# joesharratt1229/DT4Image_Restoration

Hardware: AMD Instinct MI355X
Metric: pnp_admm_iterations_per_sec (higher is better)
Workload: dtype f32

## Files before the change

### dt4image_restoration_amd/csrc/conv_kernels.hip

```cpp
#include "pnp_internal.h"
#include "conv_staging.h"
#include <cstring>
#include <cstdlib>

namespace pnp {



const LayerSpec kLayers[N_LAYERS] = {
    {2, 32, 3, 0, SRC_SIGMA, 0},    {32, 32, 3, 0, SRC_PLAIN, 0},   {32, 32, 3, 0, SRC_PLAIN, 0},
    {32, 64, 3, 1, SRC_POOL, 0},    {64, 64, 3, 1, SRC_PLAIN, 0},   {64, 64, 3, 1, SRC_PLAIN, 0},
    {64, 128, 3, 2, SRC_POOL, 0},   {128, 128, 3, 2, SRC_PLAIN, 0}, {128, 128, 3, 2, SRC_PLAIN, 0},
    {128, 256, 3, 3, SRC_POOL, 0},  {256, 256, 3, 3, SRC_PLAIN, 0}, {256, 256, 3, 3, SRC_PLAIN, 0},
    {256, 512, 3, 4, SRC_POOL, 0},  {512, 512, 3, 4, SRC_PLAIN, 0}, {512, 512, 3, 4, SRC_PLAIN, 0},
    {768, 256, 3, 3, SRC_UPCAT, 256}, {256, 256, 3, 3, SRC_PLAIN, 0}, {256, 256, 3, 3, SRC_PLAIN, 0},
    {384, 128, 3, 2, SRC_UPCAT, 128}, {128, 128, 3, 2, SRC_PLAIN, 0}, {128, 128, 3, 2, SRC_PLAIN, 0},
    {192, 64, 3, 1, SRC_UPCAT, 64},  {64, 64, 3, 1, SRC_PLAIN, 0},   {64, 64, 3, 1, SRC_PLAIN, 0},
    {96, 32, 3, 0, SRC_UPCAT, 32},   {32, 32, 3, 0, SRC_PLAIN, 0},   {32, 32, 3, 0, SRC_PLAIN, 0},
    {32, 1, 1, 0, SRC_PLAIN, 0},
};

ConvPlan conv3x3_plan(int N, int H, int W, int Cin, int Cout, bool bf16, int src_mode, bool allow_ws) {
    ConvPlan p{};
    p.tw = W >= 32 ? 32 : (W >= 16 ? 16 : 8);
// ... 613 lines not shown
    if (blocks > 2048u) blocks = 2048u;
    hipLaunchKernelGGL(splitk_reduce_kernel, dim3(blocks), dim3(256), 0, s, a.partial, a.bias, a.dst, a.tact, plane4,
                       p.splitk, a.Cout / 4, (size_t)a.H * a.W * a.Cout / 4);
    return hipGetLastError();
}

bool conv3x3_tensor_fits(int N, int H, int W, int Cin, int Cout) {
    (void)Cin;
    return (size_t)N * H * W * (size_t)Cout * 4 < ((size_t)1 << 31);
}

bool conv3x3_pooled_output_ok(const ConvPlan& p) {
    return p.splitk == 1 && p.mt <= 2 && p.nt == 1 && p.wm == 4;
}

size_t conv3x3_partial_floats(const ConvPlan& p, int N, int H, int W, int Cout) {
    return (p.mt <= 2 && p.wn >= 2) ? (size_t)p.splitk * N * H * W * Cout : 0;
}

Tuning tuning_from_env() {
    Tuning t;
    if (const char* v = getenv("PNP_WINO_MIN_CIN")) t.wino_min_cin = atoi(v);
    if (const char* v = getenv("PNP_WINO_MIN_BLOCKS")) t.wino_min_blocks = atol(v);
    t.wino_big = getenv("PNP_WINO_BIG_GROUPS") != nullptr;
    t.wino_small = getenv("PNP_WINO_SMALL_GROUPS") != nullptr;
    t.no_wino = getenv("PNP_NO_WINOGRAD") != nullptr;
    if (const char* v = getenv("PNP_WINO_F4_MIN_CIN")) t.f4_min_cin = atoi(v);
    t.no_f4 = getenv("PNP_NO_WINO_F4") != nullptr;
    t.no_f4_phased = getenv("PNP_NO_WINO_F4_PHASED") != nullptr;
    t.no_f4_fused_last = getenv("PNP_NO_F4_FUSED_LAST") != nullptr;
    t.no_f4_fused_first = getenv("PNP_NO_F4_FUSED_FIRST") != nullptr;
    if (const char* v = getenv("PNP_WINO_F4_MT16")) t.f4_mt16 = atoi(v);
    if (const char* v = getenv("PNP_WINO_F4_CS")) t.f4_cs = atoi(v);
    if (const char* v = getenv("PNP_WINO_F4_ORDER")) t.f4_order = atoi(v) != 0;
    t.bf16_f32_acts = getenv("PNP_BF16_F32_ACTS") != nullptr;
    t.bf16_no_ws = getenv("PNP_BF16_NO_WS") != nullptr;
    t.bf16_w1 = getenv("PNP_BF16_W1") != nullptr;
    t.bf16_no_holdhi = getenv("PNP_BF16_NO_HOLDHI") != nullptr;
    if (const char* v = getenv("PNP_SLICE128_MIN_N")) t.slice128_min_n = atoi(v);
    if (const char* v = getenv("PNP_TV_NAIVE")) t.tv_naive = atoi(v) != 0;
    if (const char* v = getenv("PNP_HAAR_NAIVE")) t.haar_naive = atoi(v) != 0;
    if (const char* v = getenv("PNP_NCSENSE_COIL_BLOCK")) t.ncsense_block = atoi(v);
    if (const char* v = getenv("PNP_NCSENSE_NAIVE")) t.ncsense_naive = atoi(v) != 0 ? 1 : 0;
    if (const char* v = getenv("PNP_TOEPLITZ_NAIVE")) t.toeplitz_naive = atoi(v) != 0;
    if (const char* v = getenv("PNP_OFFRES_SEG_BLOCK")) t.offres_block = atoi(v);
    if (const char* v = getenv("PNP_OFFRES_GRID_FILTER")) t.offres_grid_filter = atoi(v) != 0;
    if (const char* v = getenv("PNP_FIELDMAP_NAIVE")) t.fieldmap_naive = atoi(v) != 0;
    if (const char* v = getenv("PNP_OFFRES_NAIVE")) t.offres_naive = atoi(v) != 0 ? 1 : 0;
    return t;
}

hipError_t raise_lds_cap(const void* fn, int bytes, DeviceOnce& once) {
    int dev = 0;
    hipError_t e = hipGetDevice(&dev);
    if (e != hipSuccess) return e;
    const uint64_t bit = 1ull << (dev & 63);
    if (once.mask.load(std::memory_order_relaxed) & bit) return hipSuccess;
    e = hipFuncSetAttribute(fn, hipFuncAttributeMaxDynamicSharedMemorySize, bytes);
    if (e != hipSuccess) return e;
    once.mask.fetch_or(bit, std::memory_order_relaxed);
    return hipSuccess;
}

__global__ __launch_bounds__(256) void conv_first_kernel(const float* __restrict__ ximg, const float2* __restrict__ z,
                                                         const float2* __restrict__ u, const float* __restrict__ sigma,
                                                         const float* __restrict__ tact, const float* __restrict__ w,
// ... 172 lines not shown
```

### dt4image_restoration_amd/csrc/pnp_internal.h

```cpp
#pragma once
#include <hip/hip_runtime.h>
#include <stdint.h>
#include <stddef.h>
#include <atomic>
#include <vector>

namespace pnp {

struct Tuning {
    int wino_min_cin = 32;
    long wino_min_blocks = 192;
    bool wino_big = false;
    bool wino_small = false;
    bool no_wino = false;
    int f4_min_cin = 32;
    bool no_f4 = false;
    bool no_f4_fused_first = false;
    bool no_f4_fused_last = false;
    bool no_f4_phased = false;
    int f4_mt16 = 0;
    bool bf16_no_ws = false;
    bool bf16_f32_acts = false;
    bool bf16_no_holdhi = false;
    bool bf16_w1 = false;
    int f4_cs = 1;
    int f4_order = 1;
    int slice128_min_n = 192;
    bool tv_naive = false;
    bool haar_naive = false;
    int ncsense_block = 0;
    int ncsense_naive = -1;
    bool toeplitz_naive = false;
    int offres_block = 0;
    bool offres_grid_filter = false;
    bool fieldmap_naive = false;
    int offres_naive = -1;
};
Tuning tuning_from_env();

struct DeviceOnce { std::atomic<uint64_t> mask{0}; };
hipError_t raise_lds_cap(const void* fn, int bytes, DeviceOnce& once);

enum SrcMode : int { SRC_PLAIN = 0, SRC_SIGMA = 1, SRC_POOL = 2, SRC_UPCAT = 3, SRC_FIRST = 4 };

struct LayerSpec {
    int cin, cout, ksize, level, src, cskip;
};
static constexpr int N_LAYERS = 28;
extern const LayerSpec kLayers[N_LAYERS];

struct ConvArgs {
    const float* src0;
    const float* src1;
    const float* wpack;
    const float* bias;
    float* dst;
    float* pooled;
    const float* last_w; const float* last_b; const float* last_ximg; const float2* last_z; const float2* last_u; float* last_out;
// ... 14 lines not shown
    int diag;
#endif
};

struct ConvPlan {
    int tw, th;
    int bm, bn;
    int mt, nt, wm, wn;
    int ck;
    int splitk;
    int ws;
    int holdhi = 1;
    int tiles_x, tiles_y;
};
ConvPlan conv3x3_plan(int N, int H, int W, int Cin, int Cout, bool bf16 = false, int src_mode = SRC_PLAIN, bool allow_ws = true);
hipError_t launch_conv3x3_bf16ws(const ConvArgs& a, const ConvPlan& p, int src_mode, hipStream_t s);
size_t conv3x3_partial_floats(const ConvPlan& p, int N, int H, int W, int Cout);
bool conv3x3_pooled_output_ok(const ConvPlan& p);
bool conv3x3_tensor_fits(int N, int H, int W, int Cin, int Cout);
hipError_t launch_conv3x3(const ConvArgs& a, const ConvPlan& p, int src_mode, hipStream_t s);

size_t conv3x3_pack_floats(int cin, int cout);
void pack_conv3x3_weights(const float* oihw, int cin, int cout, int ck, float* dst);
size_t conv3x3_pack_floats_bf16(int cin, int cout, int terms);
void pack_conv3x3_weights_bf16(const float* oihw, int cin, int cout, int ck, int terms, float* dst);

struct WinoPlan {
    bool use;
    int algo;
    int tw, th, bn, wm, wn, ck, tiles_x, tiles_y;
    int stack;
    int mt;
    int phased;
    int cs;
    int order;
};
WinoPlan winograd_plan(int N, int H, int W, int Cin, int Cout, int src_mode, const Tuning& t, int Cskip = 0);
bool upsample_lines_regular(int H);
size_t winograd4_pack_floats(int cin, int cout);
void pack_winograd4_weights(const float* oihw, int cin, int cout, int ck, float* dst);
hipError_t launch_conv3x3_winograd4(const ConvArgs& a, const WinoPlan& p, int src_mode, hipStream_t s);
size_t winograd_pack_floats(int cin, int cout);
void pack_winograd_weights(const float* oihw, int cin, int cout, int ck, float* dst);
hipError_t launch_conv3x3_winograd(const ConvArgs& a, const WinoPlan& p, int src_mode, hipStream_t s);

hipError_t launch_conv_first(const float* ximg, const float2* z, const float2* u, const float* sigma,
                             const float* tact, const float* w, const float* bias, float* dst,
                             int N, int H, int W, hipStream_t s, bool dst_bf16 = false);
hipError_t launch_conv_last(const float* act, const float* ximg, const float2* z, const float2* u,
                            const float* tact, const float* w, const float* bias, float* out,
                            int N, int H, int W, hipStream_t s);
hipError_t launch_nhwc_to_nchw(const float* src, float* dst, int N, int C, int H, int W, hipStream_t s);

struct FftPlan {
    int h, w;
    float2* tw_h;
    float2* tw_w;
};

bool kspace_len_ok(int L);
hipError_t launch_fft_rows(const float2* in, float2* out, const float2* tw, int batch, int H, int W, int inverse, int shift, hipStream_t s);
hipError_t launch_fft_cols(float2* data, const float2* tw, int batch, int H, int W, int inverse, int shift, hipStream_t s);
hipError_t launch_fft_rows_real(const float* x, float2* work, const float2* tw, int N, int H, int W, hipStream_t s);
hipError_t launch_fft_rows_fwd_admm(const float* x, const float2* u, float2* work, const float2* tw, const float* tact, int N, int H, int W,
                                    hipStream_t s);
hipError_t launch_fft_cols_prox(float2* work, const float2* tw, const float2* y0s, const uint8_t* masks, int mask_n, const float* mu,
// ... 254 lines not shown
```

### dt4image_restoration_amd/csrc/winograd4_kernels.hip

```cpp
#include "pnp_internal.h"
#include "conv_staging.h"
#include <type_traits>

namespace pnp {

#ifdef PNP_STAMPS
#define W4_SLOTS 32
#define W4_WGS 1024
#define W4_N 16
__device__ unsigned long long g_w4_stamps[W4_SLOTS * W4_WGS * W4_N];
static int g_w4_slot = 0;
#define W4T() __builtin_amdgcn_s_memtime()
#endif

namespace {
constexpr double kA = 0.75, kB = 1.5;
constexpr float fA = 0.75f, fB = 1.5f, fA2 = 0.5625f, fB2 = 2.25f, fA3 = 0.421875f, fB3 = 3.375f;
constexpr float fK0 = 1.265625f;
constexpr float fK1 = 2.8125f;

__device__ __forceinline__ float4 f4add(float4 a, float4 b) { return make_float4(a.x + b.x, a.y + b.y, a.z + b.z, a.w + b.w); }
typedef float v2f __attribute__((ext_vector_type(2)));
typedef float f32x4 __attribute__((ext_vector_type(4)));

// ... 160 lines not shown
    const int g = (isrow ? ty0 : tx0) + pq - 1;
    float4 e = make_float4(0.f, 0.f, 0.f, 0.f);
    if (g >= 0 && g < (isrow ? a.H : a.W)) {
        const float sc = (isrow ? a.rh : a.rw) * (float)g;
        const int i0 = (int)sc;
        const int i1 = i0 + (i0 < (isrow ? Hs : Ws) - 1 ? 1 : 0);
        const float l = fminf(fmaxf(sc - (float)i0, 0.f), 1.f);
        if (isrow) {
            const int s0 = ylo + (pq >> 1);
            const float w0 = 1.f - l, w1 = l;
            e.x = (i0 == s0 ? w0 : 0.f) + (i1 == s0 ? w1 : 0.f);
            e.y = (i0 == s0 + 1 ? w0 : 0.f) + (i1 == s0 + 1 ? w1 : 0.f);
        } else {
            e = make_float4(__int_as_float((i0 - xlo) * LP), __int_as_float((i1 - xlo) * LP), 1.f - l, l);
        }
    }
    *reinterpret_cast<float4*>(&(isrow ? rowT : colT)[4 * pq]) = e;
}

template <int CTRL>
__device__ __forceinline__ float dpp_xchg(float v) {
    return __builtin_bit_cast(float, __builtin_amdgcn_update_dpp(0, __builtin_bit_cast(int, v), CTRL, 0xF, 0xF, false));
}
template <int H, int CTRL>
__device__ __forceinline__ void row_reduce_scatter_step(v2f* P, bool bit) {
#pragma unroll
    for (int i = 0; i < H; ++i) {
        const v2f lo = P[i], hi = P[i + H];
        const v2f keep = bit ? hi : lo, send = bit ? lo : hi;
        P[i] = v2f{keep.x + dpp_xchg<CTRL>(send.x), keep.y + dpp_xchg<CTRL>(send.y)};
    }
}

template <int TW, bool STK, int MT = 32, bool FUSE = false>
__device__ __forceinline__ void wino4_epilogue(const ConvArgs& a, const f32x4 (&acc)[36], int n, int th, int tg, int cl, int cb,
                                               int tx0, int ty0, bool live, float* xch = nullptr) {
    constexpr int TC = TW / 4, TR = MT / TC;
    constexpr unsigned OOB = 0x80000000u;
    const int cout0 = cb * 16 + cl;
    const float bias = a.bias[cout0];
    const int Hp = a.H >> 1, Wp = a.W >> 1;
    auto at6 = [&](v2f m0, v2f m1, v2f m2, v2f m3, v2f m4, v2f m5, v2f* t) {
        const v2f s1 = m1 + m2, d1 = m1 - m2, s2 = m3 + m4, d2 = m3 - m4;
        t[0] = m0 + s1 + s2;
        t[1] = fA * d1 + fB * d2;
        t[2] = fA2 * s1 + fB2 * s2;
        t[3] = fA3 * d1 + fB3 * d2 + m5;
    };
    if (!live) return;
    const bool fused = FUSE && a.last_w != nullptr;
#ifdef PNP_DIAG
    const bool nostore = (a.diag & 1) != 0;
#else
    constexpr bool nostore = false;
#endif
    v2f part[2];
    const __amdgpu_buffer_rsrc_t rdst = __builtin_amdgcn_make_buffer_rsrc(
        (void*)(a.dst + (size_t)(n + (STK ? th : 0)) * a.H * a.W * a.Cout), 0, nostore ? 0 : a.H * a.W * a.Cout * 4, 0x00020000);
    const __amdgpu_buffer_rsrc_t rpool = __builtin_amdgcn_make_buffer_rsrc(
        (void*)(a.pooled != nullptr ? a.pooled + (size_t)(n + (STK ? th : 0)) * Hp * Wp * a.Cout : a.dst), 0,
        (a.pooled != nullptr && !nostore) ? Hp * Wp * a.Cout * 4 : 0, 0x00020000);
#pragma unroll
    for (int rp = 0; rp < 2; ++rp) {
        v2f T[4][6];
#pragma unroll
        for (int j = 0; j < 6; ++j) {
            v2f m[6];
#pragma unroll
            for (int i = 0; i < 6; ++i) m[i] = v2f{acc[6 * i + j][2 * rp], acc[6 * i + j][2 * rp + 1]};
            v2f t[4];
            at6(m[0], m[1], m[2], m[3], m[4], m[5], t);
#pragma unroll
            for (int ay = 0; ay < 4; ++ay) T[ay][j] = t[ay];
        }
        v2f Y[4][4];
#pragma unroll
        for (int ay = 0; ay < 4; ++ay) {
            at6(T[ay][0], T[ay][1], T[ay][2], T[ay][3], T[ay][4], T[ay][5], Y[ay]);
#pragma unroll
            for (int ax = 0; ax < 4; ++ax) {
                const v2f sv = Y[ay][ax] + bias;
                Y[ay][ax] = v2f{fmaxf(sv.x, kLeaky * sv.x), fmaxf(sv.y, kLeaky * sv.y)};
            }
        }
        if constexpr (FUSE) {
            if (fused) {
                const float wl = a.last_w[cout0];
                v2f P[16];
#pragma unroll
                for (int i = 0; i < 16; ++i) P[i] = Y[i >> 2][i & 3] * wl;
                row_reduce_scatter_step<8, 0x140>(P, (cl & 8) != 0);
                row_reduce_scatter_step<4, 0x141>(P, (cl & 4) != 0);
                row_reduce_scatter_step<2, 0x1B>(P, (cl & 2) != 0);
                row_reduce_scatter_step<1, 0xB1>(P, (cl & 1) != 0);
                part[rp] = P[0];
                continue;
            }
        }
#pragma unroll
        for (int e = 0; e < 2; ++e) {
            const int t = 16 * th + 4 * tg + 2 * rp + e;
            const int tr = t / TC;
            const int py = STK ? 4 * (tr % (TR / 2)) : 4 * tr, px = 4 * (t % TC);
            const int gy = ty0 + py, gx = tx0 + px;
            const unsigned base = (gx < a.W) ? (unsigned)(((gy * a.W + gx) * a.Cout + cout0) * 4) : OOB;
            const unsigned rowb = (unsigned)(a.W * a.Cout * 4);
#pragma unroll
// ... 12 lines not shown
#pragma unroll
                    for (int wx = 0; wx < 2; ++wx) {
                        const v2f mx = __builtin_elementwise_max(__builtin_elementwise_max(Y[2 * wy][2 * wx], Y[2 * wy][2 * wx + 1]),
                                                                 __builtin_elementwise_max(Y[2 * wy + 1][2 * wx], Y[2 * wy + 1][2 * wx + 1]));
                        const float val = e == 0 ? mx.x : mx.y;
                        __builtin_amdgcn_raw_buffer_store_b32(__builtin_bit_cast(unsigned, val), rpool, pbase + wy * prowb, wx * a.Cout * 4, 0);
                    }
            }
        }
    }
    if constexpr (FUSE) {
        if (fused) {
            const int cq = cb & 1, lane = 16 * tg + cl;
            float4* const x4 = reinterpret_cast<float4*>(xch) + th * 64 + lane;
            if (cq == 1) *x4 = make_float4(part[0].x, part[0].y, part[1].x, part[1].y);
            __syncthreads();
            if (cq == 0) {
                const float4 o = *x4;
                const float sum[4] = {part[0].x + o.x, part[0].y + o.y, part[1].x + o.z, part[1].y + o.w};
                const float lb = a.last_b[0];
#pragma unroll
                for (int r = 0; r < 4; ++r) {
                    const int t = 16 * th + 4 * tg + r;
                    const int gy = ty0 + 4 * (t / TC) + (cl >> 2), gx = tx0 + 4 * (t % TC) + (cl & 3);
                    if (gy < a.H && gx < a.W && !nostore) {
                        const size_t qx = ((size_t)n * a.H + gy) * a.W + gx;
                        const float img = a.last_ximg != nullptr ? a.last_ximg[qx] : (a.last_z[qx].x - a.last_u[qx].x);
                        a.last_out[qx] = fminf(fmaxf(img + sum[r] + lb, 0.f), 1.f);
                    }
                }
            }
        }
    }
}

template <int TW, int SRC, bool STK = false, int WN = 2, int MT = 32>
__global__ __launch_bounds__(8 * MT * WN, 2) void conv3x3_wino4_kernel(const ConvArgs a) {
    constexpr int CK = 8 * WN, CKP = CK, LP = CK, PPP = CK / 4, NT_ = 8 * MT * WN;
    constexpr int CKQ = WN == 2 ? CK + 4 : CK + 2;
    constexpr int HCN = CK / 2;
    constexpr int TC = TW / 4, TR = MT / TC;
    constexpr int TH = 4 * TR;
    constexpr int SUBH = STK ? TH / 2 + 2 : 0;
    constexpr int PH = STK ? 2 * SUBH : TH + 2, PW = TW + 2;
    constexpr int ITEMS = PH * PW * PPP;
    static_assert(!STK || (TW == 16 && SRC == SRC_PLAIN && WN == 2 && MT == 32), "stacked slices: 16-wide tiles, plain source");
    static_assert(MT == 32 || (MT == 16 && WN == 2), "16-tile M-blocks: 64-channel workgroups only");
    constexpr int NIT = (ITEMS + NT_ - 1) / NT_;
    constexpr bool UP2 = SRC == SRC_UPCAT;
    constexpr bool FIRST = SRC == SRC_FIRST;
    constexpr int LH = TH / 2 + 3, LW = TW / 2 + 3;
    constexpr int LITEMS = LH * LW * PPP;
    constexpr int NITL = (LITEMS + NT_ - 1) / NT_;
    constexpr bool SPLIT = UP2 && WN == 2;
    constexpr int NH0 = SPLIT ? (NIT + 1) / 2 : NIT;
    constexpr int NRAW = SPLIT ? (NH0 > NITL ? NH0 : NITL) : ((UP2 && NITL > NIT) ? NITL : NIT);
    constexpr int S = CK / 4;
    constexpr int PF = WN == 2 ? 9 : 12;
    constexpr int KEEP = WN == 1 ? 6 : 3;
    constexpr int PLANE = MT * CKP;
    static_assert(SRC == SRC_PLAIN || SRC == SRC_UPCAT || SRC == SRC_FIRST, "pooled sources go through the pooled copy");
    static_assert(!FIRST || (WN == 1 && MT == 32), "fused first layer: the 32-channel variant");
    static_assert(36 % PF == 0 && MT * HCN * 2 == NT_, "one (tile, 2-channel, column group) transform item per thread");

    extern __shared__ __attribute__((aligned(16))) float smem[];
    float* const patch = smem;
// ... 291 lines not shown
            }
#ifdef PNP_DIAG
            if ((a.diag & 4) && (xi & 1)) continue;
#endif
            if (xi + PF < 36 + KEEP) bq[xi % PF] = bfrag(bp, bf0, xi + PF);
        }
#ifdef PNP_STAMPS
        { const unsigned long long t = W4T(); st_mfma += t - st_tmp; }
#endif
        if (c + 1 < nchunks) {
            if constexpr (FIRST) first_patch(c + 1);
            else park(c + 1, SPLIT ? 1 : 0);
        }
    }
#ifdef PNP_STAMPS
    st_loop1 = W4T();
    st_tmp = st_loop1;
#endif

    wino4_epilogue<TW, STK, MT, WN == 1 && MT == 32 && SRC == SRC_PLAIN>(a, acc, n, th, tg, cl, cb, tx0, ty0, STK ? (th == 0 ? live0 : live1) : true, smem);
#ifdef PNP_STAMPS
    {
        const int w = (int)blockIdx.x - (int)(gridDim.x / 2);
        if (tid == 0 && w >= 0 && w < W4_WGS && a.stamp_slot < W4_SLOTS) {
            unsigned long long* o = g_w4_stamps + ((size_t)a.stamp_slot * W4_WGS + w) * W4_N;
            const unsigned long long te = W4T();
            o[0] = 1; o[1] = st_setup - st_t0; o[2] = st_commit; o[3] = st_trans; o[4] = st_mfma; o[5] = st_loop1 - st_loop0;
            o[6] = te - st_tmp; o[7] = 0; o[8] = te - st_loop1; o[9] = te - st_t0; o[10] = (unsigned long long)nchunks;
        }
    }
#endif
}

template <int TW, bool STK>
__global__ __launch_bounds__(512, 2) void conv3x3_wino4p_kernel(const ConvArgs a) {
    constexpr int CK = 16, CKP = 16, PPP = 4, NT_ = 512, S = 4;
    constexpr int TC = TW / 4, TR = 32 / TC;
    constexpr int TH = 4 * TR;
    constexpr int SUBH = STK ? TH / 2 + 2 : 0;
    constexpr int PH = STK ? 2 * SUBH : TH + 2, PW = TW + 2;
    constexpr int NPIX = PH * PW, ITEMS = NPIX * PPP;
    constexpr int NIT = (ITEMS + NT_ - 1) / NT_;
    constexpr int PLSZ = ((NPIX * 4 + 15) / 16) * 16 + 4;
    constexpr int PATCH = 4 * PLSZ;
    constexpr int PF = 12, KEEP = 3;
    constexpr int PLANE = 32 * CKP;
    constexpr unsigned OOB = 0x80000000u;
    static_assert(!STK || TW == 16, "stacked slices: 16-wide tiles");
    static_assert((2 * PATCH + 36 * PLANE) * 4 <= 160 * 1024, "two patch copies + V in one CU's LDS");

    extern __shared__ __attribute__((aligned(16))) float smem[];
    float* const patch = smem;
    float* const V = smem + 2 * PATCH;
#ifdef PNP_STAMPS
    unsigned long long st_t0 = W4T(), st_setup = 0, st_loop0 = 0, st_commit = 0, st_trans = 0, st_mfma = 0, st_loop1 = 0, st_tmp = 0;
#endif
    const int tid = threadIdx.x, lane = tid & 63;
    const int wid = __builtin_amdgcn_readfirstlane(tid >> 6);
    const int grp = wid >> 2, cq = wid & 3;
    const int th = grp;
    const int tg = lane >> 4, cl = lane & 15;

    const int ny = a.Cout / 64;
    const int bid = blockIdx.x;
    const int ntl = a.tilesX * a.tilesY * (STK ? (a.N + 1) / 2 : a.N);
    int cby, bt;
    wino4_decode(bid, ny, ntl, a.order, cby, bt);
    if (bt >= ntl) return;
    const int tx0 = (bt % a.tilesX) * TW;
    bt /= a.tilesX;
    const int ty0 = (bt % a.tilesY) * TH;
    const int n = STK ? 2 * (bt / a.tilesY) : bt / a.tilesY;
    const int nsl = STK ? (n + 1 < a.N ? 2 : 1) : 1;
    const bool live0 = !(a.tact != nullptr && a.tact[n] > 0.5f);
    const bool live1 = STK && nsl == 2 && !(a.tact != nullptr && a.tact[n + 1] > 0.5f);
    if (!live0 && !live1) return;
    const int cb = cby * 4 + cq;
    const int nchunks = a.Cin / CK;

    const __amdgpu_buffer_rsrc_t rsrc0 = __builtin_amdgcn_make_buffer_rsrc(
        (void*)(a.src0 + (size_t)n * a.H * a.W * a.Cin), 0, nsl * a.H * a.W * a.Cin * 4, 0x00020000);
    unsigned voff[NIT];
#pragma unroll
    for (int k = 0; k < NIT; ++k) {
        const int idx = tid + k * NT_;
        const int part = idx % PPP, pp = idx / PPP;
        const int py = pp / PW, px = pp % PW;
        const int sub = STK ? py / SUBH : 0;
        const int gy = STK ? py % SUBH - 1 : ty0 + py - 1, gx = tx0 + px - 1;
        voff[k] = (idx < ITEMS && sub < nsl && gy >= 0 && gy < a.H && gx >= 0 && gx < a.W)
                      ? (unsigned)((((sub * a.H + gy) * a.W + gx) * a.Cin + part * 4) * 4) : OOB;
    }
    const int ldst = (tid & 3) * PLSZ + (tid >> 2) * 4;
    float4 raw[NIT];
    auto issue = [&](int c) {
        const int soff = c * CK * 4;
#pragma unroll
        for (int k = 0; k < NIT; ++k)
            raw[k] = __builtin_bit_cast(float4, __builtin_amdgcn_raw_buffer_load_b128(rsrc0, voff[k], soff, 0));
    };
    auto park = [&](int c) {
        float* const dst = patch + (c & 1) * PATCH + ldst;
#pragma unroll
        for (int k = 0; k < NIT; ++k)
            if (tid + k * NT_ < ITEMS) *reinterpret_cast<float4*>(&dst[k * (NT_ / PPP) * 4]) = raw[k];
    };

    auto swz = [](int t16, int g) { return g ^ ((4 - (t16 >> 2)) & 3); };
    const int tgi = tid & 255;
    const int hc = tgi & 7, t16 = (tgi >> 3) & 15;
    const int tj = (wid >> 1) & 1;
    const int tq = 16 * grp + t16;
    const int trow = tq / TC;
    const int wrow = STK ? (trow / (TR / 2)) * SUBH + 4 * (trow % (TR / 2)) : 4 * trow;
    const int win = (hc >> 1) * PLSZ + (wrow * PW + 4 * (tq % TC)) * 4 + 2 * (hc & 1);
    const int vout = tq * CKP + 4 * swz(t16, hc >> 1) + 2 * (hc & 1);

    f32x4 acc[36];
#pragma unroll
    for (int k = 0; k < 36; ++k) acc[k] = f32x4{0.f, 0.f, 0.f, 0.f};

    const size_t stream = (size_t)nchunks * 36 * 64 + kW4Tail / S;
    const float4* const bptr = reinterpret_cast<const float4*>(a.wpack) + (size_t)cb * stream + lane;
    float4 bq[PF];
#pragma unroll
    for (int p = 0; p < KEEP; ++p) bq[p] = bptr[p * 64];
    const int aoff = (16 * th + cl) * CKP + 4 * swz(cl, tg);

    constexpr bool PARK_T = !STK;
    issue(0);
    park(0);
    if constexpr (!PARK_T) { if (grp == 1 && nchunks > 1) { issue(1); park(1); } }
#ifdef PNP_STAMPS
    st_setup = W4T();
    st_loop0 = st_setup;
#endif
    if (grp == 1) __syncthreads();
    for (int c = 0; c < nchunks; ++c) {
#ifdef PNP_STAMPS
        st_tmp = W4T();
#endif
        __syncthreads();
#ifdef PNP_STAMPS
        { const unsigned long long t = W4T(); st_commit += t - st_tmp; st_tmp = t; }
#endif
        if constexpr (PARK_T) { if (c + 1 < nchunks) issue(c + 1); }
        __builtin_amdgcn_s_setprio(3);
        {
            const float* const w = patch + (c & 1) * PATCH + win;
            if (tj == 0) wino4_input_transform<0, PW, 4, PLANE>(w, V + vout);
            else wino4_input_transform<1, PW, 4, PLANE>(w, V + vout);
        }
        __builtin_amdgcn_s_setprio(0);
        __builtin_amdgcn_sched_barrier(0);
        const float4* bp = bptr + (size_t)c * 36 * 64;
#pragma unroll
        for (int p = KEEP; p < PF; ++p) bq[p] = bp[p * 64];
        const int nx = c + 1 + grp;
        if constexpr (PARK_T) { if (c + 1 < nchunks) park(c + 1); }
        else { if (nx < nchunks) issue(nx); }
        __syncthreads();
#ifdef PNP_STAMPS
        { const unsigned long long t = W4T(); st_trans += t - st_tmp; st_tmp = t; }
#endif

        float4 ar[3];
        ar[0] = *reinterpret_cast<const float4*>(&V[aoff]);
        ar[1] = *reinterpret_cast<const float4*>(&V[PLANE + aoff]);
#pragma unroll
        for (int xi = 0; xi < 36; ++xi) {
            if (xi + 2 < 36) ar[(xi + 2) % 3] = *reinterpret_cast<const float4*>(&V[(xi + 2) * PLANE + aoff]);
            __builtin_amdgcn_sched_barrier(0);
            const float4 a0 = ar[xi % 3], b0 = bq[xi % PF];
            acc[xi] = __builtin_amdgcn_mfma_f32_16x16x4f32(a0.x, b0.x, acc[xi], 0, 0, 0);
            acc[xi] = __builtin_amdgcn_mfma_f32_16x16x4f32(a0.y, b0.y, acc[xi], 0, 0, 0);
            acc[xi] = __builtin_amdgcn_mfma_f32_16x16x4f32(a0.z, b0.z, acc[xi], 0, 0, 0);
            acc[xi] = __builtin_amdgcn_mfma_f32_16x16x4f32(a0.w, b0.w, acc[xi], 0, 0, 0);
            __builtin_amdgcn_sched_barrier(0);
#ifdef PNP_DIAG
            if ((a.diag & 4) && (xi & 1)) continue;
#endif
            if (xi + PF < 36 + KEEP) bq[xi % PF] = bp[(xi + PF) * 64];
        }
#ifdef PNP_STAMPS
        { const unsigned long long t = W4T(); st_mfma += t - st_tmp; }
#endif
        if constexpr (!PARK_T) { if (nx < nchunks) park(nx); }
    }
    if (grp == 0) __syncthreads();
#ifdef PNP_STAMPS
    st_loop1 = W4T();
    st_tmp = st_loop1;
#endif

    wino4_epilogue<TW, STK>(a, acc, n, th, tg, cl, cb, tx0, ty0, STK ? (th == 0 ? live0 : live1) : true);
#ifdef PNP_STAMPS
    {
        const int w = (int)blockIdx.x - (int)(gridDim.x / 2);
        if (tid == 0 && w >= 0 && w < W4_WGS && a.stamp_slot < W4_SLOTS) {
            unsigned long long* o = g_w4_stamps + ((size_t)a.stamp_slot * W4_WGS + w) * W4_N;
            const unsigned long long te = W4T();
            o[0] = 1; o[1] = st_setup - st_t0; o[2] = st_commit; o[3] = st_trans; o[4] = st_mfma; o[5] = st_loop1 - st_loop0;
            o[6] = te - st_tmp; o[7] = 0; o[8] = te - st_loop1; o[9] = te - st_t0; o[10] = (unsigned long long)nchunks;
        }
    }
#endif
}

template <int TW, int SRC>
__global__ __launch_bounds__(512, 2) void conv3x3_wino4c_kernel(const ConvArgs a) {
    constexpr int CK = 16, CKP = 16, PPP = 4, NT_ = 512, S = 4, MT = 16;
    constexpr bool UP2 = SRC == SRC_UPCAT;
    static_assert(SRC == SRC_PLAIN || SRC == SRC_UPCAT, "plain or upsample + concat source");
    constexpr int TC = TW / 4, TR = MT / TC;
    constexpr int TH = 4 * TR;
    constexpr int PH = TH + 2, PW = TW + 2;
    constexpr int NPIX = PH * PW, ITEMS = NPIX * PPP;
    constexpr int NIT = (ITEMS + NT_ - 1) / NT_;
    constexpr int PLSZ = ((NPIX * 4 + 15) / 16) * 16 + 4;
    constexpr int PATCH = 4 * PLSZ;
    constexpr int PF = 12, KEEP = 3;
    constexpr int PLANE = MT * CKP;
    constexpr int VSZ = 36 * PLANE;
    constexpr unsigned OOB = 0x80000000u;
    static_assert(NIT == 3 && ITEMS <= NIT * NT_, "three staging items per thread");
    constexpr int LP = CK;
    constexpr int LH = TH / 2 + 3, LW = TW / 2 + 3;
    constexpr int LITEMS = LH * LW * PPP, NITL = (LITEMS + NT_ - 1) / NT_;
// ... 200 lines not shown

    wino4_epilogue<TW, false, 16>(a, acc, n, 0, tg, cl, cb, tx0, ty0, true);
#ifdef PNP_STAMPS
    {
        const int w = (int)blockIdx.x - (int)(gridDim.x / 2);
        if (tid == 0 && w >= 0 && w < W4_WGS && a.stamp_slot < W4_SLOTS) {
            unsigned long long* o = g_w4_stamps + ((size_t)a.stamp_slot * W4_WGS + w) * W4_N;
            const unsigned long long te = W4T();
            o[0] = 1; o[1] = st_setup - st_t0; o[2] = st_commit; o[3] = st_trans; o[4] = st_mfma; o[5] = st_loop1 - st_loop0;
            o[6] = te - st_tmp; o[7] = 0; o[8] = te - st_loop1; o[9] = te - st_t0; o[10] = (unsigned long long)nchunks;
        }
    }
#endif
}

template <int TW, int SRC>
static hipError_t launch_wino4c_inst(const ConvArgs& a, const WinoPlan& p, hipStream_t s) {
    constexpr int TC = TW / 4, TR = 16 / TC, TH = 4 * TR;
    constexpr int NPIX = (TH + 2) * (TW + 2);
    constexpr int PLSZ = ((NPIX * 4 + 15) / 16) * 16 + 4;
    constexpr size_t lowres_f = SRC == SRC_UPCAT ? (size_t)2 * (TH / 2 + 3) * (TW / 2 + 3) * 16 + 4 * (TH + 2 + TW + 2) : 0;
    constexpr size_t lds = ((size_t)2 * 4 * PLSZ + (size_t)2 * 36 * 16 * 16 + lowres_f) * sizeof(float);
    if (p.th != TH || p.tw != TW) return hipErrorInvalidValue;
    if (SRC == SRC_UPCAT && a.Cskip < 3 * 16) return hipErrorInvalidValue;
    auto kern = conv3x3_wino4c_kernel<TW, SRC>;
    static DeviceOnce cap;
    if (hipError_t e = raise_lds_cap((const void*)kern, (int)lds, cap); e != hipSuccess) return e;
    const int ntiles = p.tiles_x * p.tiles_y * a.N, ny = a.Cout / 128;
    dim3 grid((unsigned)(((ntiles + 7) / 8) * 8 * ny));
    hipLaunchKernelGGL(kern, grid, dim3(512), lds, s, a);
    return hipGetLastError();
}

template <int TW, bool STK>
static hipError_t launch_wino4p_inst(const ConvArgs& a, const WinoPlan& p, hipStream_t s) {
    constexpr int TC = TW / 4, TR = 32 / TC, TH = 4 * TR;
    constexpr int NPIX = (STK ? TH + 4 : TH + 2) * (TW + 2);
    constexpr int PLSZ = ((NPIX * 4 + 15) / 16) * 16 + 4;
    constexpr size_t lds = ((size_t)2 * 4 * PLSZ + (size_t)36 * 32 * 16) * sizeof(float);
    auto kern = conv3x3_wino4p_kernel<TW, STK>;
    static DeviceOnce cap;
    if (hipError_t e = raise_lds_cap((const void*)kern, (int)lds, cap); e != hipSuccess) return e;
    const int ntiles = p.tiles_x * p.tiles_y * (STK ? (a.N + 1) / 2 : a.N), ny = a.Cout / 64;
    dim3 grid((unsigned)(((ntiles + 7) / 8) * 8 * ny));
    hipLaunchKernelGGL(kern, grid, dim3(512), lds, s, a);
    return hipGetLastError();
}

template <int TW, int SRC, bool STK = false, int WN = 2, int MT = 32>
static hipError_t launch_wino4_inst(const ConvArgs& a, const WinoPlan& p, hipStream_t s) {
    constexpr int CK = 8 * WN, CKP = CK, CKQ = WN == 2 ? CK + 4 : CK + 2, TC = TW / 4, TR = MT / TC, TH = 4 * TR;
    constexpr size_t patch_f = (((size_t)(STK ? TH + 4 : TH + 2) * (TW + 2) * CKQ + 3) / 4) * 4;
    constexpr size_t lowres_f = SRC == SRC_UPCAT ? (size_t)(TH / 2 + 3) * (TW / 2 + 3) * CK + 4 * (TH + 2 + TW + 2) : 0;
    constexpr size_t first_f = SRC == SRC_FIRST ? (size_t)2 * (TH + 4) * (TW + 5) + 18 * 32 + 64 : 0;
    constexpr size_t lds = (patch_f + (size_t)36 * MT * CKP + lowres_f + first_f) * sizeof(float);
    static_assert(lds <= (WN == 2 && MT == 32 ? 160 : 80) * 1024, "one (8 waves) / two (4 waves) workgroups per CU");
    if (p.th != TH || p.tw != TW) return hipErrorInvalidValue;
    auto kern = conv3x3_wino4_kernel<TW, SRC, STK, WN, MT>;
    static DeviceOnce cap;
    if (hipError_t e = raise_lds_cap((const void*)kern, (int)lds, cap); e != hipSuccess) return e;
    const int ntiles = p.tiles_x * p.tiles_y * (STK ? (a.N + 1) / 2 : a.N), ny = a.Cout / (32 * WN);
    dim3 grid((unsigned)(((ntiles + 7) / 8) * 8 * ny));
    hipLaunchKernelGGL(kern, grid, dim3(8 * MT * WN), lds, s, a);
    return hipGetLastError();
}

hipError_t launch_conv3x3_winograd4(const ConvArgs& a0, const WinoPlan& p, int src_mode, hipStream_t s) {
    if (!p.use || p.algo != 4 || a0.Cout % p.bn || a0.Cin % p.ck || (src_mode == SRC_UPCAT && a0.Cskip % p.ck) || a0.W % 4) return hipErrorInvalidValue;
    if (a0.last_w != nullptr && !(p.bn == 32 && p.mt == 32 && src_mode == SRC_PLAIN)) return hipErrorInvalidValue;
    ConvArgs a = a0;
    a.tilesX = p.tiles_x;
    a.tilesY = p.tiles_y;
    a.order = p.order;
#ifdef PNP_STAMPS
    a.stamp_slot = g_w4_slot++;
#endif
    if (p.bn == 32) {
        if (p.ck != 8 || p.stack) return hipErrorInvalidValue;
        if (p.tw == 32 && src_mode == SRC_PLAIN) return launch_wino4_inst<32, SRC_PLAIN, false, 1>(a, p, s);
        if (p.tw == 32 && src_mode == SRC_UPCAT) return launch_wino4_inst<32, SRC_UPCAT, false, 1>(a, p, s);
        if (p.tw == 32 && src_mode == SRC_FIRST) return launch_wino4_inst<32, SRC_FIRST, false, 1>(a, p, s);
        if (p.tw == 16 && src_mode == SRC_FIRST) return launch_wino4_inst<16, SRC_FIRST, false, 1>(a, p, s);
        if (p.tw == 16 && src_mode == SRC_PLAIN) return launch_wino4_inst<16, SRC_PLAIN, false, 1>(a, p, s);
        if (p.tw == 16 && src_mode == SRC_UPCAT) return launch_wino4_inst<16, SRC_UPCAT, false, 1>(a, p, s);
        return hipErrorInvalidValue;
    }
    if (p.ck != 16) return hipErrorInvalidValue;
    if (p.cs) {
        if (p.bn != 128 || p.mt != 16 || p.stack) return hipErrorInvalidValue;
        if (p.tw == 32 && src_mode == SRC_PLAIN) return launch_wino4c_inst<32, SRC_PLAIN>(a, p, s);
        if (p.tw == 32 && src_mode == SRC_UPCAT) return launch_wino4c_inst<32, SRC_UPCAT>(a, p, s);
        if (p.tw == 16 && src_mode == SRC_PLAIN) return launch_wino4c_inst<16, SRC_PLAIN>(a, p, s);
        if (p.tw == 16 && src_mode == SRC_UPCAT) return launch_wino4c_inst<16, SRC_UPCAT>(a, p, s);
        return hipErrorInvalidValue;
    }
    if (p.mt == 16) {
        if (p.stack) return hipErrorInvalidValue;
        if (p.tw == 32 && src_mode == SRC_PLAIN) return launch_wino4_inst<32, SRC_PLAIN, false, 2, 16>(a, p, s);
        if (p.tw == 32 && src_mode == SRC_UPCAT) return launch_wino4_inst<32, SRC_UPCAT, false, 2, 16>(a, p, s);
        if (p.tw == 16 && src_mode == SRC_PLAIN) return launch_wino4_inst<16, SRC_PLAIN, false, 2, 16>(a, p, s);
        if (p.tw == 16 && src_mode == SRC_UPCAT) return launch_wino4_inst<16, SRC_UPCAT, false, 2, 16>(a, p, s);
        return hipErrorInvalidValue;
    }
    if (p.phased && src_mode == SRC_PLAIN) {
        if (p.tw == 32 && !p.stack) return launch_wino4p_inst<32, false>(a, p, s);
        if (p.tw == 16) {
            if (p.stack) return a.H == 16 && a.W == 16 ? launch_wino4p_inst<16, true>(a, p, s) : hipErrorInvalidValue;
            return launch_wino4p_inst<16, false>(a, p, s);
        }
        return hipErrorInvalidValue;
    }
    if (p.tw == 32) {
        if (src_mode == SRC_PLAIN) return launch_wino4_inst<32, SRC_PLAIN>(a, p, s);
        if (src_mode == SRC_UPCAT) return launch_wino4_inst<32, SRC_UPCAT>(a, p, s);
    } else if (p.tw == 16) {
        if (p.stack) return src_mode == SRC_PLAIN && a.H == 16 && a.W == 16 ? launch_wino4_inst<16, SRC_PLAIN, true>(a, p, s) : hipErrorInvalidValue;
        if (src_mode == SRC_PLAIN) return launch_wino4_inst<16, SRC_PLAIN>(a, p, s);
        if (src_mode == SRC_UPCAT) return launch_wino4_inst<16, SRC_UPCAT>(a, p, s);
    }
    return hipErrorInvalidValue;
}

}

#ifdef PNP_STAMPS
extern "C" int pnp_debug_stamps4_reset(void) { pnp::g_w4_slot = 0; return 0; }
extern "C" int pnp_debug_stamps4_read(unsigned long long* dst, int slots) {
    return (int)hipMemcpyFromSymbol(dst, HIP_SYMBOL(pnp::g_w4_stamps), (size_t)slots * W4_WGS * W4_N * sizeof(unsigned long long));
}
#endif
```

### dt4image_restoration_amd/csrc/winograd_kernels.hip

```cpp
#include "pnp_internal.h"
#include "conv_staging.h"
#include <cstdlib>

namespace pnp {

#ifdef PNP_STAMPS
#define PNP_STAMP_SLOTS 32
#define PNP_STAMP_WGS 1024
#define PNP_STAMP_N 112
__device__ unsigned long long g_wino_stamps[PNP_STAMP_SLOTS * PNP_STAMP_WGS * PNP_STAMP_N];
static int g_stamp_slot = 0;
#define STAMP() do { if (ns < PNP_STAMP_N) st[ns] = __builtin_amdgcn_s_memtime(); ++ns; } while (0)
#else
#define STAMP() do { } while (0)
#endif

size_t winograd_pack_floats(int cin, int cout) { return (size_t)(cout / 32) * ((size_t)(cin / 8) * 16 * 256 + 2 * 4 * 256); }

void pack_winograd_weights(const float* oihw, int cin, int cout, int ck, float* dst) {
    static const double G[4][3] = {{1, 0, 0}, {0.5, 0.5, 0.5}, {0.5, -0.5, 0.5}, {0, 0, 1}};
    std::vector<float> U((size_t)cout * cin * 16);
    for (int co = 0; co < cout; ++co)
        for (int ci = 0; ci < cin; ++ci) {
            const float* g = oihw + ((size_t)co * cin + ci) * 9;
// ... 34 lines not shown
        WinoPlan f{};
        f.algo = 4;
        f.order = (t.f4_order && (long)H * W >= 32 * 32) ? 1 : 0;
        f.tw = W >= 32 ? 32 : 16;
        f.th = f.tw == 32 ? 16 : 32;
        f.bn = 64; f.wm = 1; f.wn = 2; f.ck = 16;
        if (Cout == 32) { f.bn = 32; f.wn = 1; f.ck = 8; }
        f.tiles_x = (W + f.tw - 1) / f.tw;
        f.tiles_y = (H + f.th - 1) / f.th;
        f.stack = (W == 16 && H == 16) ? 1 : 0;
        if (!(f.stack && Cout == 32)) {
            f.mt = 32;
            const bool mt16 = t.f4_mt16 == 0 ? (src_mode == SRC_UPCAT || Cin <= 64) : (t.f4_mt16 == 1 ? false : (t.f4_mt16 == 2 ? src_mode == SRC_UPCAT : true));
            if (f.bn == 64 && mt16 && (f.tw == 32 ? H >= 8 : H >= 16)) {
                f.mt = 16;
                f.th = f.tw == 32 ? 8 : 16;
                f.tiles_y = (H + f.th - 1) / f.th;
                f.stack = 0;
            }
            f.phased = (f.mt == 32 && f.bn == 64 && src_mode == SRC_PLAIN && !t.no_f4_phased) ? 1 : 0;
            const bool cs_can = f.bn == 64 && Cout % 128 == 0 && (src_mode == SRC_PLAIN || (Cskip % 16 == 0 && Cskip >= 48));
            const int cs_th = f.tw == 32 ? 8 : 16;
            const long cs_blocks = (long)f.tiles_x * ((H + cs_th - 1) / cs_th) * N * (Cout / 128);
            const bool cs_rule = src_mode == SRC_UPCAT && cs_blocks >= kCsMinBlocks;
            if (cs_can && cs_blocks >= t.wino_min_blocks && (t.f4_cs == 2 || (t.f4_cs == 1 && t.f4_mt16 == 0 && !t.no_f4_phased && cs_rule))) {
                f.cs = 1;
                f.bn = 128;
                f.mt = 16;
                f.th = cs_th;
                f.tiles_y = (H + f.th - 1) / f.th;
                f.stack = 0;
                f.phased = 0;
            }
            const long blocks = (long)f.tiles_x * f.tiles_y * (f.stack ? (N + 1) / 2 : N) * (Cout / f.bn);
            f.use = blocks >= t.wino_min_blocks;
            if (f.use) return f;
        }
    }
    p.tw = W >= 32 ? 32 : (W >= 16 ? 16 : 8);
    const bool big = t.wino_big;
    if (Cout % 128 == 0 && !t.wino_small) { p.wm = 1; p.wn = 4; p.ck = 32; }
    else if (Cout % 64 == 0) { if (big) { p.wm = 2; p.wn = 2; } else { p.wm = 1; p.wn = 2; } p.ck = 16; }
    else { if (big) { p.wm = 4; p.wn = 1; } else { p.wm = 2; p.wn = 1; } p.ck = 8; }
    const int tc = p.tw / 2, tr = 32 / tc;
    p.th = p.wm * 2 * tr;
    p.bn = p.wn * 32;
    p.tiles_x = (W + p.tw - 1) / p.tw;
    p.tiles_y = (H + p.th - 1) / p.th;
    const long blocks = (long)p.tiles_x * p.tiles_y * N * (Cout / p.bn);
    p.use = blocks >= t.wino_min_blocks;
    return p;
}

template <int TW, int WM, int WN, int CK, int SRC>
__global__ __launch_bounds__(WM * WN * 128, 2) void conv3x3_winograd_kernel(const ConvArgs a) {
    constexpr int GW = WM * WN;
    constexpr int NT_ = GW * 128;
    constexpr int CKP = CK + 4;
    constexpr int PPP = CK / 4;
    constexpr int TC = TW / 2, TR = 32 / TC;
    constexpr int TH = WM * 2 * TR;
    constexpr int NTILES = WM * 32;
    constexpr int PWL = TW + 2, PH = TH + 2, PW = PWL;
    constexpr int ITEMS = PH * PWL * PPP;
    constexpr int NIT = (ITEMS + NT_ - 1) / NT_;
    constexpr bool UP2 = SRC == SRC_UPCAT;
// ... 369 lines not shown
```

Measured before the change: 131.5.

## Split Winograd F4 frequency work across wave groups with LDS exchange in phased kernel

Adds an FS variant of the phased Winograd F(4,3) kernel. Each wave group takes half of the 36 transform frequencies (18) for both tile halves, rather than all 36 for one half. Each group then does half of the output transform and swaps the partial rows with the other group through LDS before the shared epilogue. The aim is to halve per-wave weight prefetch registers and B-operand streaming, reusing each weight fragment across two A tiles. The cost is an extra __syncthreads and LDS exchange traffic. It is enabled by default for phased plans with enough blocks, excluding the 128→256 layer.

```diff
diff --git a/dt4image_restoration_amd/csrc/conv_kernels.hip b/dt4image_restoration_amd/csrc/conv_kernels.hip
--- a/dt4image_restoration_amd/csrc/conv_kernels.hip
+++ b/dt4image_restoration_amd/csrc/conv_kernels.hip
@@ -669,6 +669,7 @@
     t.no_f4_fused_first = getenv("PNP_NO_F4_FUSED_FIRST") != nullptr;
     if (const char* v = getenv("PNP_WINO_F4_MT16")) t.f4_mt16 = atoi(v);
     if (const char* v = getenv("PNP_WINO_F4_CS")) t.f4_cs = atoi(v);
+    if (const char* v = getenv("PNP_WINO_F4_FS")) t.f4_fs = atoi(v);
     if (const char* v = getenv("PNP_WINO_F4_ORDER")) t.f4_order = atoi(v) != 0;
     t.bf16_f32_acts = getenv("PNP_BF16_F32_ACTS") != nullptr;
     t.bf16_no_ws = getenv("PNP_BF16_NO_WS") != nullptr;
diff --git a/dt4image_restoration_amd/csrc/pnp_internal.h b/dt4image_restoration_amd/csrc/pnp_internal.h
--- a/dt4image_restoration_amd/csrc/pnp_internal.h
+++ b/dt4image_restoration_amd/csrc/pnp_internal.h
@@ -24,6 +24,7 @@
     bool bf16_no_holdhi = false;
     bool bf16_w1 = false;
     int f4_cs = 1;
+    int f4_fs = 1;
     int f4_order = 1;
     int slice128_min_n = 192;
     bool tv_naive = false;
@@ -104,6 +105,7 @@
     int stack;
     int mt;
     int phased;
+    int fs;
     int cs;
     int order;
 };
diff --git a/dt4image_restoration_amd/csrc/winograd4_kernels.hip b/dt4image_restoration_amd/csrc/winograd4_kernels.hip
--- a/dt4image_restoration_amd/csrc/winograd4_kernels.hip
+++ b/dt4image_restoration_amd/csrc/winograd4_kernels.hip
@@ -216,21 +216,22 @@
     }
 }
 
-template <int TW, bool STK, int MT = 32, bool FUSE = false>
-__device__ __forceinline__ void wino4_epilogue(const ConvArgs& a, const f32x4 (&acc)[36], int n, int th, int tg, int cl, int cb,
-                                               int tx0, int ty0, bool live, float* xch = nullptr) {
+__device__ __forceinline__ void at6(v2f m0, v2f m1, v2f m2, v2f m3, v2f m4, v2f m5, v2f* t) {
+    const v2f s1 = m1 + m2, d1 = m1 - m2, s2 = m3 + m4, d2 = m3 - m4;
+    t[0] = m0 + s1 + s2;
+    t[1] = __builtin_elementwise_fma(v2f{fA, fA}, d1, fB * d2);
+    t[2] = __builtin_elementwise_fma(v2f{fA2, fA2}, s1, fB2 * s2);
+    t[3] = __builtin_elementwise_fma(v2f{fA3, fA3}, d1, fB3 * d2) + m5;
+}
+
+template <int TW, bool STK, int MT, bool FUSE, class Stage1>
+__device__ __forceinline__ void wino4_epilogue_from(const ConvArgs& a, Stage1 stage1, int n, int th, int tg, int cl, int cb,
+                                                    int tx0, int ty0, bool live, float* xch) {
     constexpr int TC = TW / 4, TR = MT / TC;
     constexpr unsigned OOB = 0x80000000u;
     const int cout0 = cb * 16 + cl;
     const float bias = a.bias[cout0];
     const int Hp = a.H >> 1, Wp = a.W >> 1;
-    auto at6 = [&](v2f m0, v2f m1, v2f m2, v2f m3, v2f m4, v2f m5, v2f* t) {
-        const v2f s1 = m1 + m2, d1 = m1 - m2, s2 = m3 + m4, d2 = m3 - m4;
-        t[0] = m0 + s1 + s2;
-        t[1] = fA * d1 + fB * d2;
-        t[2] = fA2 * s1 + fB2 * s2;
-        t[3] = fA3 * d1 + fB3 * d2 + m5;
-    };
     if (!live) return;
     const bool fused = FUSE && a.last_w != nullptr;
 #ifdef PNP_DIAG
@@ -247,16 +248,7 @@
 #pragma unroll
     for (int rp = 0; rp < 2; ++rp) {
         v2f T[4][6];
-#pragma unroll
-        for (int j = 0; j < 6; ++j) {
-            v2f m[6];
-#pragma unroll
-            for (int i = 0; i < 6; ++i) m[i] = v2f{acc[6 * i + j][2 * rp], acc[6 * i + j][2 * rp + 1]};
-            v2f t[4];
-            at6(m[0], m[1], m[2], m[3], m[4], m[5], t);
-#pragma unroll
-            for (int ay = 0; ay < 4; ++ay) T[ay][j] = t[ay];
-        }
+        stage1(rp, T);
         v2f Y[4][4];
 #pragma unroll
         for (int ay = 0; ay < 4; ++ay) {
@@ -335,6 +327,23 @@
             }
         }
     }
+}
+
+template <int TW, bool STK, int MT = 32, bool FUSE = false>
+__device__ __forceinline__ void wino4_epilogue(const ConvArgs& a, const f32x4 (&acc)[36], int n, int th, int tg, int cl, int cb,
+                                               int tx0, int ty0, bool live, float* xch = nullptr) {
+    wino4_epilogue_from<TW, STK, MT, FUSE>(a, [&](int rp, v2f (&T)[4][6]) {
+#pragma unroll
+        for (int j = 0; j < 6; ++j) {
+            v2f m[6];
+#pragma unroll
+            for (int i = 0; i < 6; ++i) m[i] = v2f{acc[6 * i + j][2 * rp], acc[6 * i + j][2 * rp + 1]};
+            v2f t[4];
+            at6(m[0], m[1], m[2], m[3], m[4], m[5], t);
+#pragma unroll
+            for (int ay = 0; ay < 4; ++ay) T[ay][j] = t[ay];
+        }
+    }, n, th, tg, cl, cb, tx0, ty0, live, xch);
 }
 
 template <int TW, int SRC, bool STK = false, int WN = 2, int MT = 32>
@@ -692,7 +701,7 @@
 #endif
 }
 
-template <int TW, bool STK>
+template <int TW, bool STK, bool FS = false>
 __global__ __launch_bounds__(512, 2) void conv3x3_wino4p_kernel(const ConvArgs a) {
     constexpr int CK = 16, CKP = 16, PPP = 4, NT_ = 512, S = 4;
     constexpr int TC = TW / 4, TR = 32 / TC;
@@ -703,7 +712,8 @@
     constexpr int NIT = (ITEMS + NT_ - 1) / NT_;
     constexpr int PLSZ = ((NPIX * 4 + 15) / 16) * 16 + 4;
     constexpr int PATCH = 4 * PLSZ;
-    constexpr int PF = 12, KEEP = 3;
+    constexpr int PF = FS ? 6 : 12, KEEP = 3;
+    constexpr int NF = FS ? 18 : 36;
     constexpr int PLANE = 32 * CKP;
     constexpr unsigned OOB = 0x80000000u;
     static_assert(!STK || TW == 16, "stacked slices: 16-wide tiles");
@@ -769,8 +779,8 @@
     auto swz = [](int t16, int g) { return g ^ ((4 - (t16 >> 2)) & 3); };
     const int tgi = tid & 255;
     const int hc = tgi & 7, t16 = (tgi >> 3) & 15;
-    const int tj = (wid >> 1) & 1;
-    const int tq = 16 * grp + t16;
+    const int tj = FS ? grp : (wid >> 1) & 1;
+    const int tq = FS ? tgi >> 3 : 16 * grp + t16;
     const int trow = tq / TC;
     const int wrow = STK ? (trow / (TR / 2)) * SUBH + 4 * (trow % (TR / 2)) : 4 * trow;
     const int win = (hc >> 1) * PLSZ + (wrow * PW + 4 * (tq % TC)) * 4 + 2 * (hc & 1);
@@ -781,11 +791,13 @@
     for (int k = 0; k < 36; ++k) acc[k] = f32x4{0.f, 0.f, 0.f, 0.f};
 
     const size_t stream = (size_t)nchunks * 36 * 64 + kW4Tail / S;
-    const float4* const bptr = reinterpret_cast<const float4*>(a.wpack) + (size_t)cb * stream + lane;
+    auto fo = [](int k) { return FS ? (k / NF) * 36 * 64 + (6 * ((k % NF) / 3) + k % 3) * 64 : k * 64; };
+    const float4* const bptr = reinterpret_cast<const float4*>(a.wpack) + (size_t)cb * stream + lane + (FS ? 3 * grp * 64 : 0);
     float4 bq[PF];
 #pragma unroll
-    for (int p = 0; p < KEEP; ++p) bq[p] = bptr[p * 64];
-    const int aoff = (16 * th + cl) * CKP + 4 * swz(cl, tg);
+    for (int p = 0; p < KEEP; ++p) bq[p] = bptr[fo(p)];
+    const int aoff = (16 * th + cl) * CKP + 4 * swz(cl, tg) + (FS ? 3 * grp * PLANE : 0);
+    const int aoff1 = (16 * (1 - th) + cl) * CKP + 4 * swz(cl, tg) + 3 * grp * PLANE;
 
     constexpr bool PARK_T = !STK;
     issue(0);
@@ -815,7 +827,7 @@
         __builtin_amdgcn_sched_barrier(0);
         const float4* bp = bptr + (size_t)c * 36 * 64;
 #pragma unroll
-        for (int p = KEEP; p < PF; ++p) bq[p] = bp[p * 64];
+        for (int p = KEEP; p < PF; ++p) bq[p] = bp[fo(p)];
         const int nx = c + 1 + grp;
         if constexpr (PARK_T) { if (c + 1 < nchunks) park(c + 1); }
         else { if (nx < nchunks) issue(nx); }
@@ -824,6 +836,37 @@
         { const unsigned long long t = W4T(); st_trans += t - st_tmp; st_tmp = t; }
 #endif
 
+        if constexpr (FS) {
+        auto vp = [](int k) { return (6 * (k / 3) + k % 3) * PLANE; };
+        float4 ar[3][2];
+#pragma unroll
+        for (int k = 0; k < 2; ++k) {
+            ar[k][0] = *reinterpret_cast<const float4*>(&V[vp(k) + aoff]);
+            ar[k][1] = *reinterpret_cast<const float4*>(&V[vp(k) + aoff1]);
+        }
+#pragma unroll
+        for (int k = 0; k < NF; ++k) {
+            if (k + 2 < NF) {
+                ar[(k + 2) % 3][0] = *reinterpret_cast<const float4*>(&V[vp(k + 2) + aoff]);
+                ar[(k + 2) % 3][1] = *reinterpret_cast<const float4*>(&V[vp(k + 2) + aoff1]);
+            }
+            __builtin_amdgcn_sched_barrier(0);
+            const float4 a0 = ar[k % 3][0], a1 = ar[k % 3][1], b0 = bq[k % PF];
+            acc[k] = __builtin_amdgcn_mfma_f32_16x16x4f32(a0.x, b0.x, acc[k], 0, 0, 0);
+            acc[k] = __builtin_amdgcn_mfma_f32_16x16x4f32(a0.y, b0.y, acc[k], 0, 0, 0);
+            acc[k] = __builtin_amdgcn_mfma_f32_16x16x4f32(a0.z, b0.z, acc[k], 0, 0, 0);
+            acc[k] = __builtin_amdgcn_mfma_f32_16x16x4f32(a0.w, b0.w, acc[k], 0, 0, 0);
+            acc[NF + k] = __builtin_amdgcn_mfma_f32_16x16x4f32(a1.x, b0.x, acc[NF + k], 0, 0, 0);
+            acc[NF + k] = __builtin_amdgcn_mfma_f32_16x16x4f32(a1.y, b0.y, acc[NF + k], 0, 0, 0);
+            acc[NF + k] = __builtin_amdgcn_mfma_f32_16x16x4f32(a1.z, b0.z, acc[NF + k], 0, 0, 0);
+            acc[NF + k] = __builtin_amdgcn_mfma_f32_16x16x4f32(a1.w, b0.w, acc[NF + k], 0, 0, 0);
+            __builtin_amdgcn_sched_barrier(0);
+#ifdef PNP_DIAG
+            if ((a.diag & 4) && (k & 1)) continue;
+#endif
+            if (k + PF < NF + KEEP) bq[k % PF] = bp[fo(k + PF)];
+        }
+        } else {
         float4 ar[3];
         ar[0] = *reinterpret_cast<const float4*>(&V[aoff]);
         ar[1] = *reinterpret_cast<const float4*>(&V[PLANE + aoff]);
@@ -842,6 +885,7 @@
 #endif
             if (xi + PF < 36 + KEEP) bq[xi % PF] = bp[(xi + PF) * 64];
         }
+        }
 #ifdef PNP_STAMPS
         { const unsigned long long t = W4T(); st_mfma += t - st_tmp; }
 #endif
@@ -853,7 +897,60 @@
     st_tmp = st_loop1;
 #endif
 
+    if constexpr (FS) {
+        static_assert(2 * PATCH >= 12288 + 4 * 6 * 256, "exchange slots in the patch space");
+        v2f own[2][4][3], oth[2][4][3];
+#pragma unroll
+        for (int rp = 0; rp < 2; ++rp)
+#pragma unroll
+            for (int j = 0; j < 3; ++j) {
+                v2f m[6], t[4];
+#pragma unroll
+                for (int i = 0; i < 6; ++i) m[i] = v2f{acc[3 * i + j][2 * rp], acc[3 * i + j][2 * rp + 1]};
+                at6(m[0], m[1], m[2], m[3], m[4], m[5], t);
+#pragma unroll
+                for (int ay = 0; ay < 4; ++ay) own[rp][ay][j] = t[ay];
+#pragma unroll
+                for (int i = 0; i < 6; ++i) m[i] = v2f{acc[NF + 3 * i + j][2 * rp], acc[NF + 3 * i + j][2 * rp + 1]};
+                at6(m[0], m[1], m[2], m[3], m[4], m[5], t);
+#pragma unroll
+                for (int ay = 0; ay < 4; ++ay) oth[rp][ay][j] = t[ay];
+            }
+        auto xlo = [&](int g) { return g == 0 ? smem + cq * 12 * 256 : smem + 12288 + cq * 6 * 256; };
+        auto xhi = [&](int g) { return g == 0 ? smem + cq * 12 * 256 + 6 * 256 : V + cq * 6 * PLANE; };
+        {
+            float* const lo = xlo(grp) + lane * 4;
+            float* const hi = xhi(grp) + lane * 4;
+#pragma unroll
+            for (int q = 0; q < 12; ++q) {
+                const v2f e0 = oth[(2 * q) / 12][((2 * q) / 3) % 4][(2 * q) % 3], e1 = oth[(2 * q + 1) / 12][((2 * q + 1) / 3) % 4][(2 * q + 1) % 3];
+                *reinterpret_cast<float4*>((q < 6 ? lo : hi) + (q % 6) * 256) = make_float4(e0.x, e0.y, e1.x, e1.y);
+            }
+        }
+        __syncthreads();
+        v2f rcv[2][4][3];
+        {
+            const float* const lo = xlo(1 - grp) + lane * 4;
+            const float* const hi = xhi(1 - grp) + lane * 4;
+#pragma unroll
+            for (int q = 0; q < 12; ++q) {
+                const float4 r = *reinterpret_cast<const float4*>((q < 6 ? lo : hi) + (q % 6) * 256);
+                rcv[(2 * q) / 12][((2 * q) / 3) % 4][(2 * q) % 3] = v2f{r.x, r.y};
+                rcv[(2 * q + 1) / 12][((2 * q + 1) / 3) % 4][(2 * q + 1) % 3] = v2f{r.z, r.w};
+            }
+        }
+        wino4_epilogue_from<TW, STK, 32, false>(a, [&](int rp, v2f (&T)[4][6]) {
+#pragma unroll
+            for (int ay = 0; ay < 4; ++ay)
+#pragma unroll
+                for (int j = 0; j < 3; ++j) {
+                    T[ay][j] = grp == 0 ? own[rp][ay][j] : rcv[rp][ay][j];
+                    T[ay][3 + j] = grp == 0 ? rcv[rp][ay][j] : own[rp][ay][j];
+                }
+        }, n, th, tg, cl, cb, tx0, ty0, STK ? (th == 0 ? live0 : live1) : true, nullptr);
+    } else {
     wino4_epilogue<TW, STK>(a, acc, n, th, tg, cl, cb, tx0, ty0, STK ? (th == 0 ? live0 : live1) : true);
+    }
 #ifdef PNP_STAMPS
     {
         const int w = (int)blockIdx.x - (int)(gridDim.x / 2);
@@ -1120,13 +1217,13 @@
     return hipGetLastError();
 }
 
-template <int TW, bool STK>
+template <int TW, bool STK, bool FS = false>
 static hipError_t launch_wino4p_inst(const ConvArgs& a, const WinoPlan& p, hipStream_t s) {
     constexpr int TC = TW / 4, TR = 32 / TC, TH = 4 * TR;
     constexpr int NPIX = (STK ? TH + 4 : TH + 2) * (TW + 2);
     constexpr int PLSZ = ((NPIX * 4 + 15) / 16) * 16 + 4;
     constexpr size_t lds = ((size_t)2 * 4 * PLSZ + (size_t)36 * 32 * 16) * sizeof(float);
-    auto kern = conv3x3_wino4p_kernel<TW, STK>;
+    auto kern = conv3x3_wino4p_kernel<TW, STK, FS>;
     static DeviceOnce cap;
     if (hipError_t e = raise_lds_cap((const void*)kern, (int)lds, cap); e != hipSuccess) return e;
     const int ntiles = p.tiles_x * p.tiles_y * (STK ? (a.N + 1) / 2 : a.N), ny = a.Cout / 64;
@@ -1191,10 +1288,11 @@
         return hipErrorInvalidValue;
     }
     if (p.phased && src_mode == SRC_PLAIN) {
-        if (p.tw == 32 && !p.stack) return launch_wino4p_inst<32, false>(a, p, s);
+        if (p.tw == 32 && !p.stack) return p.fs ? launch_wino4p_inst<32, false, true>(a, p, s) : launch_wino4p_inst<32, false>(a, p, s);
         if (p.tw == 16) {
-            if (p.stack) return a.H == 16 && a.W == 16 ? launch_wino4p_inst<16, true>(a, p, s) : hipErrorInvalidValue;
-            return launch_wino4p_inst<16, false>(a, p, s);
+            if (p.stack && !(a.H == 16 && a.W == 16)) return hipErrorInvalidValue;
+            if (p.stack) return p.fs ? launch_wino4p_inst<16, true, true>(a, p, s) : launch_wino4p_inst<16, true>(a, p, s);
+            return p.fs ? launch_wino4p_inst<16, false, true>(a, p, s) : launch_wino4p_inst<16, false>(a, p, s);
         }
         return hipErrorInvalidValue;
     }
diff --git a/dt4image_restoration_amd/csrc/winograd_kernels.hip b/dt4image_restoration_amd/csrc/winograd_kernels.hip
--- a/dt4image_restoration_amd/csrc/winograd_kernels.hip
+++ b/dt4image_restoration_amd/csrc/winograd_kernels.hip
@@ -90,6 +90,10 @@
                 f.stack = 0;
                 f.phased = 0;
             }
+            constexpr long kFsMinBlocks = 256;
+            const long fs_blocks = (long)f.tiles_x * f.tiles_y * (f.stack ? (N + 1) / 2 : N) * (Cout / 64);
+            const bool fs_rule = fs_blocks >= kFsMinBlocks && !(Cin == 128 && Cout == 256);
+            f.fs = (f.phased && (t.f4_fs == 2 || (t.f4_fs == 1 && fs_rule))) ? 1 : 0;
             const long blocks = (long)f.tiles_x * f.tiles_y * (f.stack ? (N + 1) / 2 : N) * (Cout / f.bn);
             f.use = blocks >= t.wino_min_blocks;
             if (f.use) return f;
```

New measurement: 132.5, median of 6. No clear change (+0.8%).
